# DrownFish19/PaddleXDE

Measured on AMD Instinct MI355X. Metric: integrated states/sec (batch*dim/step_time) dopri5, higher is better.
Workload: dtype f32

## Files before the change

paddlexde_amd/csrc/xde_seam.hip:

```cpp

#include "xde_common.hpp"
#include "xde_reduce.hpp"
#include "xde_errnorm_device.hpp"
#include "xde_control_device.hpp"
#include "xde_hip_seam.h"

using namespace xde;

namespace {

constexpr int kSeamCap = XDE_SEAM_CAP;
constexpr int kSeamBatch = 4;
constexpr int kSeamBlocksPerCU = 2;
static_assert(kSeamCap % kSeamBatch == 0, "whole batches");

struct alignas(128) SeamLine {
  unsigned long long gen;
  unsigned long long pad[15];
};
struct SeamState {
  SeamLine line[kTicketShards];
  SeamLine expired;
};

struct SeamCtrl {
  xde_ctrl_t* ctrl;
  xde_ctrl_params_t p;
  const double* t_span;
  const double* step_t;
  void* t_stage_out;
  xde_ctrl_t* mirror;
  int flags;
};

struct SeamArgs {
  ErrArgs e;
  const void* f0[2];
  void* out;
  double a21;
  SeamState* st;
  long long spin_limit;
};

template <typename T, int NORM, bool NT>
__global__ __launch_bounds__(kBlock, kSeamBlocksPerCU) void xde_seam_kernel(SeamArgs s, SeamCtrl tl) {
  __shared__ double seg_val[XDE_MAX_SEG];
  __shared__ double seg_nf[XDE_MAX_SEG];
  __shared__ xde_ctrl_t zs;
  __shared__ TimePrefetch pfs;
  __shared__ xde_ctrl_t sink;
  __shared__ double t_sink[XDE_MAX_STAGE];
  __shared__ int s_expired;
  using P = Pack<T, true>;
  constexpr int W = P::W;
  const ErrArgs& a = s.e;
  const bool pub = blockIdx.x == 0;
  control_prologue(tl.ctrl, tl.p, tl.t_span, tl.step_t, pub ? tl.mirror : nullptr, tl.flags, &zs, &pfs);

  const T* epre = static_cast<const T*>(a.e_pre);
  const T* __restrict__ kl = static_cast<const T*>(a.k[0]);
  const T* __restrict__ y1 = static_cast<const T*>(a.y1);
  const int64_t start = a.map.seg_start[0];
  const int64_t len = a.map.seg_len[0];
  const int64_t nvec = len / W;
  const int64_t vbase = start / W;
  const int64_t stride = int64_t(gridDim.x) * kBlock;
  const int64_t b0 = int64_t(blockIdx.x) * kBlock;
  const int64_t i0 = b0 + threadIdx.x;
  const double dtd = __builtin_nontemporal_load(&a.ctrl->dt);
  const int32_t accw = __builtin_nontemporal_load(&a.ctrl->accept);
  unsigned long long prior = 0;
  if (threadIdx.x == 0) prior = __hip_atomic_load(&s.st->expired.gen, __ATOMIC_RELAXED, __HIP_MEMORY_SCOPE_AGENT);
  const T rtol = T(a.rtol), atol = T(a.atol);
  const int sel = (a.use_sel && accw) ? 1 : 0;
  const T* __restrict__ y0 = static_cast<const T*>(a.y0[sel]);
  const T c = T(dtd) * T(a.coef[0]);
  T acc = T(0);
  int nfw = 0;
  P cy[kSeamCap], ck[kSeamCap];
  auto one = [&](bool on, T e, T y0e, T y1e) {
    T tol = atol + rtol * fmax_(abs_(y0e), abs_(y1e));
    T ar = abs_(e / tol);
    if (on) {
      if (NORM == XDE_NORM_RMS) {
        acc = acc + ar * ar;
      } else {
        acc = (ar != ar || acc != acc) ? (ar != ar ? ar : acc) : (ar > acc ? ar : acc);
      }
    }
    nfw += __popcll(__ballot(on && nonfinite_class(y0e)));
  };
#pragma unroll
  for (int jb = 0; jb < kSeamCap; jb += kSeamBatch) {
    if (b0 + int64_t(jb) * stride < nvec) {
      P ep[kSeamBatch], yv[kSeamBatch];
#pragma unroll
      for (int u = 0; u < kSeamBatch; ++u) {
        const int64_t i = i0 + int64_t(jb + u) * stride;
        const int64_t ic = vbase + (i < nvec ? i : nvec - 1);
        cy[jb + u] = P::load(y1, ic);
        ep[u] = NT ? P::load_nt(epre, ic) : P::load(epre, ic);
        ck[jb + u] = P::load(kl, ic);
        yv[u] = NT ? P::load_nt(y0, ic) : P::load(y0, ic);
      }
#pragma unroll
      for (int u = 0; u < kSeamBatch; ++u) {
        const bool on = i0 + int64_t(jb + u) * stride < nvec;
#pragma unroll
        for (int w = 0; w < W; ++w) one(on, ep[u].v[w] + ck[jb + u].v[w] * c, yv[u].v[w], cy[jb + u].v[w]);
      }
    }
  }
  const int64_t tj = start + nvec * W + threadIdx.x;
  const bool ton = blockIdx.x == 0 && tj < start + len;
  T ty1 = T(1), tk = T(0);
  if (blockIdx.x == 0) {
    T e = T(0), y0e = T(0);
    if (ton) {
      tk = kl[tj];
      e = epre[tj] + tk * c;
      y0e = y0[tj];
      ty1 = y1[tj];
    }
    if (ton) {
      T tol = atol + rtol * fmax_(abs_(y0e), abs_(ty1));
      T ar = abs_(e / tol);
      if (NORM == XDE_NORM_RMS) acc = acc + ar * ar;
      else acc = (ar != ar || acc != acc) ? (ar != ar ? ar : acc) : (ar > acc ? ar : acc);
    }
    nfw += __popcll(__ballot(ton && nonfinite_class(y0e)));
  }
  const double acc_d = NORM == XDE_NORM_RMS ? 0.0 + double(acc) : double(acc);
  const double nf_d = (threadIdx.x & 63) == 0 ? double(nfw) : 0.0;
  if (blockIdx.x == 0 && threadIdx.x == 0) {
    a.slot->nblocks = gridDim.x;
    a.slot->n_seg = 1;
    a.slot->norm_kind = NORM;
  }
  const bool last = block_reduce_store<NORM, true>(acc_d, nf_d, a.slot, 0);

  const unsigned long long tag = (unsigned long long)(zs.seq + 1);
  if (last) {
    if (threadIdx.x < kTicketShards)
      __hip_atomic_store(&a.slot->shard[threadIdx.x].count, 0u, __ATOMIC_RELAXED, __HIP_MEMORY_SCOPE_AGENT);
    if (threadIdx.x == 0) __hip_atomic_store(&a.slot->ticket, 0u, __ATOMIC_RELAXED, __HIP_MEMORY_SCOPE_AGENT);
    if (threadIdx.x < kTicketShards)
      __hip_atomic_store(&s.st->line[threadIdx.x].gen, tag, __ATOMIC_RELAXED, __HIP_MEMORY_SCOPE_AGENT);
  }
  if (threadIdx.x == 0) {
    int expired = prior != 0 ? 1 : 0;
    if (!last) {
      const unsigned nsh = gridDim.x < unsigned(kTicketShards) ? gridDim.x : unsigned(kTicketShards);
      const unsigned long long* word = &s.st->line[blockIdx.x % nsh].gen;
      long long spins = 0;
      while (__hip_atomic_load(word, __ATOMIC_RELAXED, __HIP_MEMORY_SCOPE_AGENT) != tag) {
        if (++spins > s.spin_limit) {
          expired = 1;
          unsigned long long none = 0;
          __hip_atomic_compare_exchange_strong(&s.st->expired.gen, &none, tag, __ATOMIC_RELAXED, __ATOMIC_RELAXED,
                                               __HIP_MEMORY_SCOPE_AGENT);
          break;
        }
        __builtin_amdgcn_s_sleep(8);
      }
    }
    s_expired = expired;
  }
  if (threadIdx.x < XDE_MAX_SEG) {
    seg_val[threadIdx.x] = 0.0;
    seg_nf[threadIdx.x] = 0.0;
  }
  __syncthreads();

  reduce_partials<true>(a.slot, seg_val, seg_nf, int(gridDim.x), 1, NORM);
  if (threadIdx.x == 0 && s_expired) seg_nf[0] += 1.0;
  __syncthreads();
  control_tail(pub ? tl.ctrl : &sink, tl.p, seg_val, seg_nf, tl.t_span, tl.step_t, pub ? tl.t_stage_out : static_cast<void*>(t_sink),
               pub ? tl.mirror : nullptr, tl.flags, &zs, &pfs);
  const int acc_new = zs.accept;
  const T c1 = T(s.a21) * T(zs.dt);
  T* out = static_cast<T*>(s.out);
  if (acc_new) {
#pragma unroll
    for (int j = 0; j < kSeamCap; ++j) {
      const int64_t i = i0 + int64_t(j) * stride;
      if (i < nvec) {
        P o;
#pragma unroll
        for (int w = 0; w < W; ++w) o.v[w] = cy[j].v[w] + ck[j].v[w] * c1;
        o.store(out, vbase + i);
      }
    }
    if (ton) out[tj] = ty1 + tk * c1;
  } else {
    const T* __restrict__ fb = static_cast<const T*>(s.f0[sel]);
    for (int64_t i = i0; i < nvec; i += stride) {
      P y = P::load(y0, vbase + i);
      P f = P::load(fb, vbase + i);
      P o;
#pragma unroll
      for (int w = 0; w < W; ++w) o.v[w] = y.v[w] + f.v[w] * c1;
      o.store(out, vbase + i);
    }
    if (ton) out[tj] = y0[tj] + fb[tj] * c1;
  }
}

template <typename T, int NORM, bool NT>
int seam_resident() {
  static int cache[64];
  static std::mutex mu;
  int dev = 0;
  if (hipGetDevice(&dev) != hipSuccess || dev < 0 || dev >= 64) {
    (void)hipGetLastError();
    return 0;
  }
  std::lock_guard<std::mutex> lk(mu);
  if (cache[dev] == 0) {
    int per_cu = 0, cus = 0;
    if (hipOccupancyMaxActiveBlocksPerMultiprocessor(&per_cu, xde_seam_kernel<T, NORM, NT>, kBlock, 0) != hipSuccess ||
        hipDeviceGetAttribute(&cus, hipDeviceAttributeMultiprocessorCount, dev) != hipSuccess) {
      (void)hipGetLastError();
      return 0;
    }
    if (per_cu > kSeamBlocksPerCU) per_cu = kSeamBlocksPerCU;
    cache[dev] = per_cu * cus > 0 ? per_cu * cus : -1;
  }
  return cache[dev] > 0 ? cache[dev] : 0;
}

int seam_resident_of(int dtype, int norm_kind, bool nt) {
#define SEAM_RES(T, NORM) (nt ? seam_resident<T, NORM, true>() : seam_resident<T, NORM, false>())
  if (dtype == XDE_F32) return norm_kind == XDE_NORM_RMS ? SEAM_RES(float, XDE_NORM_RMS) : SEAM_RES(float, XDE_NORM_LINF);
  return norm_kind == XDE_NORM_RMS ? SEAM_RES(double, XDE_NORM_RMS) : SEAM_RES(double, XDE_NORM_LINF);
#undef SEAM_RES
}

int seam_geometry(int64_t n, int dtype, int* blocks_out, int* per_lane_out) {
  xde_segments_t segs;
  memset(&segs, 0, sizeof(segs));
  segs.struct_size = sizeof(segs);
  segs.n_seg = 1;
  segs.seg_len[0] = n;
  const int width = dtype == XDE_F32 ? 4 : 2;
  SegMap m;
  int blocks = 0;
  if (int rc = build_segmap(&segs, width, true, &m, &blocks)) return rc;
  const int64_t nvec = n / width;
  const int64_t lanes = int64_t(blocks) * kBlock;
  *blocks_out = blocks;
  *per_lane_out = int((nvec + lanes - 1) / lanes);
  return XDE_OK;
}

}

extern "C" {

int64_t xde_seam_state_bytes(void) { return int64_t(sizeof(SeamState)); }

int xde_seam_plan(int64_t n, int dtype, xde_seam_plan_t* plan_out) {
  if (!plan_out) return fail(XDE_EBADARG, "xde_seam_plan: null pointer");
  if (dtype != XDE_F32 && dtype != XDE_F64) return fail(XDE_EBADARG, "xde_seam_plan: bad dtype");
  if (n < 1) return fail(XDE_EBADARG, "xde_seam_plan: n must be positive");
  memset(plan_out, 0, sizeof(*plan_out));
  int blocks = 0, per_lane = 0;
  if (int rc = seam_geometry(n, dtype, &blocks, &per_lane)) return rc;
  plan_out->blocks = blocks;
  plan_out->per_lane = per_lane;
  int resident = seam_resident_of(dtype, XDE_NORM_RMS, false);
  const int others[3] = {seam_resident_of(dtype, XDE_NORM_RMS, true), seam_resident_of(dtype, XDE_NORM_LINF, false),
                         seam_resident_of(dtype, XDE_NORM_LINF, true)};
  for (int r : others) resident = r < resident ? r : resident;
  plan_out->resident = resident;
  plan_out->fits = (blocks <= resident && per_lane <= kSeamCap) ? 1 : 0;
  return XDE_OK;
}

int xde_seam_attempt(const void* k_last, double c_last, const void* e_pre, const void* y0, const void* y0_alt, const void* f0,
                     const void* f0_alt, const void* y1, void* out, double a21, int64_t n, int dtype, void* ws, void* state,
                     xde_ctrl_t* ctrl, const xde_ctrl_params_t* params, const double* t_span_dev, const double* step_t_dev,
                     void* t_stage_out, xde_ctrl_t* host_mirror, int64_t spin_limit, void* stream) {
  if (!k_last || !e_pre || !y0 || !f0 || !y1 || !out || !ws || !state || !ctrl || !t_span_dev || !t_stage_out)
    return fail(XDE_EBADARG, "xde_seam_attempt: null pointer");
  int rc = check_params(params, "xde_seam_attempt");
  if (rc != XDE_OK) return rc;
  if (params->n_seg != 1) return fail(XDE_EBADARG, "xde_seam_attempt: one segment only");
  if (params->n_step_t > 0 && !step_t_dev) return fail(XDE_EBADARG, "xde_seam_attempt: n_step_t > 0 without step_t_dev");
  if (dtype != params->state_dtype) return fail(XDE_EBADARG, "xde_seam_attempt: dtype does not match params->state_dtype");
  if ((y0_alt == nullptr) != (f0_alt == nullptr)) return fail(XDE_EBADARG, "xde_seam_attempt: y0_alt/f0_alt must come together");
  if (n < 1) return fail(XDE_EBADARG, "xde_seam_attempt: n must be positive");
  if (spin_limit <= 0) return fail(XDE_EBADARG, "xde_seam_attempt: spin_limit must be positive (the wait is bounded)");
  xde_segments_t segs;
  memset(&segs, 0, sizeof(segs));
  segs.struct_size = sizeof(segs);
  segs.n_seg = 1;
  segs.seg_len[0] = n;
  SeamArgs s;
  memset(&s, 0, sizeof(s));
  bool vec = false;
  int nblocks = 0;
  double bytes = 0;
  const void* kk[1] = {k_last};
  rc = setup_err_args("xde_seam_attempt", kk, nullptr, &c_last, 1, y0, y0_alt, y1, params->rtol, params->atol, 0.0, ctrl, &segs,
                      params->norm_kind, dtype, ws, e_pre, &s.e, &vec, &nblocks, &bytes);
  if (rc != XDE_OK) return rc;
  vec = vec && aligned16(out) && aligned16(f0) && (!f0_alt || aligned16(f0_alt));
  if (!vec) return fail(XDE_EBADARG, "xde_seam_attempt: operands must be 16-byte aligned");
  const int width = dtype == XDE_F32 ? 4 : 2;
  const int64_t lanes = int64_t(nblocks) * kBlock;
  const int64_t per_lane = (n / width + lanes - 1) / lanes;
  const int resident = seam_resident_of(dtype, params->norm_kind, s.e.nt != 0);
  if (nblocks > resident || per_lane > kSeamCap)
    return fail(XDE_EBADARG, "xde_seam_attempt: the state does not fit the resident launch (" + std::to_string(nblocks) + " workgroups, " +
                                 std::to_string(resident) + " resident; " + std::to_string(per_lane) + " vectors per lane, " +
                                 std::to_string(kSeamCap) + " carried): take the separate launches");
  s.f0[0] = f0;
  s.f0[1] = f0_alt ? f0_alt : f0;
  s.out = out;
  s.a21 = a21;
  s.st = static_cast<SeamState*>(state);
  s.spin_limit = spin_limit;
  SeamCtrl tl;
  tl.ctrl = ctrl;
  tl.p = *params;
  tl.t_span = t_span_dev;
  tl.step_t = step_t_dev;
  tl.t_stage_out = t_stage_out;
  tl.mirror = host_mirror;
  tl.flags = ctrl_flags();
  hipStream_t st = static_cast<hipStream_t>(stream);
  ProfScope prof(XDE_KID_ERRNORM, 5.0 * double(n) * (dtype == XDE_F32 ? 4.0 : 8.0));
  dim3 g(nblocks), b(kBlock);
#define LAUNCH_SEAM(T, NORM)                                                   \
  do {                                                                         \
    if (s.e.nt)                                                                \
      XDE_LAUNCH((xde_seam_kernel<T, NORM, true>), g, b, st, prof, s, tl);     \
    else                                                                       \
      XDE_LAUNCH((xde_seam_kernel<T, NORM, false>), g, b, st, prof, s, tl);    \
  } while (0)
  if (dtype == XDE_F32) {
    if (params->norm_kind == XDE_NORM_RMS) LAUNCH_SEAM(float, XDE_NORM_RMS);
    else LAUNCH_SEAM(float, XDE_NORM_LINF);
  } else {
    if (params->norm_kind == XDE_NORM_RMS) LAUNCH_SEAM(double, XDE_NORM_RMS);
    else LAUNCH_SEAM(double, XDE_NORM_LINF);
  }
#undef LAUNCH_SEAM
  HIP_TRY(hipGetLastError());
  return XDE_OK;
}

int xde_seam_expired(const void* state, int64_t* tag_out, void* stream) {
  if (!state || !tag_out) return fail(XDE_EBADARG, "xde_seam_expired: null pointer");
  hipStream_t st = static_cast<hipStream_t>(stream);
  HIP_TRY(hipMemcpyAsync(tag_out, &static_cast<const SeamState*>(state)->expired.gen, sizeof(int64_t), hipMemcpyDeviceToHost, st));
  HIP_TRY(hipStreamSynchronize(st));
  return XDE_OK;
}

}
```

Before: 27.70 billion.

## Replace last-block ticket barrier with collector block publishing checksummed dt/accept

```diff
diff --git a/paddlexde_amd/csrc/xde_seam.hip b/paddlexde_amd/csrc/xde_seam.hip
--- a/paddlexde_amd/csrc/xde_seam.hip
+++ b/paddlexde_amd/csrc/xde_seam.hip
@@ -10,18 +10,38 @@
 namespace {
 
 constexpr int kSeamCap = XDE_SEAM_CAP;
-constexpr int kSeamBatch = 4;
+constexpr int kSeamPair = 1;
 constexpr int kSeamBlocksPerCU = 2;
-static_assert(kSeamCap % kSeamBatch == 0, "whole batches");
+constexpr int kSeamRecPer = 4;
+constexpr int kSeamCollectSleep = 1;
+static_assert(kSeamCap % kSeamPair == 0, "whole batches");
+static_assert(kSeamRecPer <= XDE_MAX_PARTIALS / kBlock, "the collector's records are reduce_records' first slots");
 
 struct alignas(128) SeamLine {
-  unsigned long long gen;
-  unsigned long long pad[15];
+  unsigned long long w[2];
+  unsigned long long pad[14];
 };
 struct SeamState {
   SeamLine line[kTicketShards];
   SeamLine expired;
 };
+
+__device__ __forceinline__ unsigned long long seam_chk(unsigned long long word, unsigned long long tag, int pos) {
+  return ctrl_mix64(word + 0x9E3779B97F4A7C15ull * (4ull * tag + (unsigned long long)pos));
+}
+
+__device__ __forceinline__ void seam_store_half(unsigned long long* at, unsigned long long word, unsigned long long tag, int pos) {
+  __hip_atomic_store(at + 0, word, __ATOMIC_RELAXED, __HIP_MEMORY_SCOPE_AGENT);
+  __hip_atomic_store(at + 1, seam_chk(word, tag, pos), __ATOMIC_RELAXED, __HIP_MEMORY_SCOPE_AGENT);
+}
+
+__device__ __forceinline__ void seam_load_half(const unsigned long long* at, unsigned long long& word, unsigned long long& check) {
+  typedef unsigned long long v2u64_t __attribute__((ext_vector_type(2)));
+  v2u64_t v;
+  asm volatile("global_load_dwordx4 %0, %1, off sc1\n\ts_waitcnt vmcnt(0)" : "=&v"(v) : "v"(at) : "memory");
+  word = v.x;
+  check = v.y;
+}
 
 struct SeamCtrl {
   xde_ctrl_t* ctrl;
@@ -48,14 +68,17 @@
   __shared__ double seg_nf[XDE_MAX_SEG];
   __shared__ xde_ctrl_t zs;
   __shared__ TimePrefetch pfs;
-  __shared__ xde_ctrl_t sink;
-  __shared__ double t_sink[XDE_MAX_STAGE];
-  __shared__ int s_expired;
+  __shared__ double s_val[kWaves];
+  __shared__ double s_nf[kWaves];
+  __shared__ int s_accept;
+  __shared__ int s_skip;
+  __shared__ unsigned long long s_dt;
+  __shared__ unsigned long long s_tag;
   using P = Pack<T, true>;
   constexpr int W = P::W;
   const ErrArgs& a = s.e;
   const bool pub = blockIdx.x == 0;
-  control_prologue(tl.ctrl, tl.p, tl.t_span, tl.step_t, pub ? tl.mirror : nullptr, tl.flags, &zs, &pfs);
+  if (pub) control_prologue(tl.ctrl, tl.p, tl.t_span, tl.step_t, tl.mirror, tl.flags, &zs, &pfs);
 
   const T* epre = static_cast<const T*>(a.e_pre);
   const T* __restrict__ kl = static_cast<const T*>(a.k[0]);
@@ -69,8 +92,11 @@
   const int64_t i0 = b0 + threadIdx.x;
   const double dtd = __builtin_nontemporal_load(&a.ctrl->dt);
   const int32_t accw = __builtin_nontemporal_load(&a.ctrl->accept);
-  unsigned long long prior = 0;
-  if (threadIdx.x == 0) prior = __hip_atomic_load(&s.st->expired.gen, __ATOMIC_RELAXED, __HIP_MEMORY_SCOPE_AGENT);
+  unsigned long long tag = 0, prior = 0;
+  if (threadIdx.x == 0) {
+    tag = (unsigned long long)(__builtin_nontemporal_load(&a.ctrl->seq) + 1);
+    prior = __hip_atomic_load(&s.st->expired.w[0], __ATOMIC_RELAXED, __HIP_MEMORY_SCOPE_AGENT);
+  }
   const T rtol = T(a.rtol), atol = T(a.atol);
   const int sel = (a.use_sel && accw) ? 1 : 0;
   const T* __restrict__ y0 = static_cast<const T*>(a.y0[sel]);
@@ -90,26 +116,45 @@
     }
     nfw += __popcll(__ballot(on && nonfinite_class(y0e)));
   };
-#pragma unroll
-  for (int jb = 0; jb < kSeamCap; jb += kSeamBatch) {
-    if (b0 + int64_t(jb) * stride < nvec) {
-      P ep[kSeamBatch], yv[kSeamBatch];
-#pragma unroll
-      for (int u = 0; u < kSeamBatch; ++u) {
-        const int64_t i = i0 + int64_t(jb + u) * stride;
-        const int64_t ic = vbase + (i < nvec ? i : nvec - 1);
-        cy[jb + u] = P::load(y1, ic);
-        ep[u] = NT ? P::load_nt(epre, ic) : P::load(epre, ic);
-        ck[jb + u] = P::load(kl, ic);
-        yv[u] = NT ? P::load_nt(y0, ic) : P::load(y0, ic);
-      }
-#pragma unroll
-      for (int u = 0; u < kSeamBatch; ++u) {
-        const bool on = i0 + int64_t(jb + u) * stride < nvec;
-#pragma unroll
-        for (int w = 0; w < W; ++w) one(on, ep[u].v[w] + ck[jb + u].v[w] * c, yv[u].v[w], cy[jb + u].v[w]);
-      }
-    }
+  P ep[2][kSeamPair], yv[2][kSeamPair];
+  auto live = [&](int jb) { return b0 + int64_t(jb) * stride < nvec; };
+  auto request = [&](int jb, int h) {
+#pragma unroll
+    for (int u = 0; u < kSeamPair; ++u) {
+      const int64_t i = i0 + int64_t(jb + u) * stride;
+      const int64_t ic = vbase + (i < nvec ? i : nvec - 1);
+      cy[jb + u] = P::load(y1, ic);
+      ep[h][u] = NT ? P::load_nt(epre, ic) : P::load(epre, ic);
+      ck[jb + u] = P::load(kl, ic);
+      yv[h][u] = NT ? P::load_nt(y0, ic) : P::load(y0, ic);
+    }
+  };
+  auto consume = [&](int jb, int h) {
+#pragma unroll
+    for (int u = 0; u < kSeamPair; ++u) {
+      const bool on = i0 + int64_t(jb + u) * stride < nvec;
+#pragma unroll
+      for (int w = 0; w < W; ++w) one(on, ep[h][u].v[w] + ck[jb + u].v[w] * c, yv[h][u].v[w], cy[jb + u].v[w]);
+    }
+  };
+  auto from = [&](auto self, auto jbc) {
+    constexpr int JB = decltype(jbc)::value;
+    constexpr int H = (JB / kSeamPair) & 1;
+    if constexpr (JB + kSeamPair < kSeamCap) {
+      if (live(JB + kSeamPair)) {
+        request(JB + kSeamPair, H ^ 1);
+        consume(JB, H);
+        self(self, std::integral_constant<int, JB + kSeamPair>{});
+      } else {
+        consume(JB, H);
+      }
+    } else {
+      consume(JB, H);
+    }
+  };
+  if (live(0)) {
+    request(0, 0);
+    from(from, std::integral_constant<int, 0>{});
   }
   const int64_t tj = start + nvec * W + threadIdx.x;
   const bool ton = blockIdx.x == 0 && tj < start + len;
@@ -130,55 +175,132 @@
     }
     nfw += __popcll(__ballot(ton && nonfinite_class(y0e)));
   }
-  const double acc_d = NORM == XDE_NORM_RMS ? 0.0 + double(acc) : double(acc);
-  const double nf_d = (threadIdx.x & 63) == 0 ? double(nfw) : 0.0;
+  double rec_v = NORM == XDE_NORM_RMS ? 0.0 + double(acc) : double(acc);
+  double rec_f = (threadIdx.x & 63) == 0 ? double(nfw) : 0.0;
   if (blockIdx.x == 0 && threadIdx.x == 0) {
     a.slot->nblocks = gridDim.x;
     a.slot->n_seg = 1;
     a.slot->norm_kind = NORM;
   }
-  const bool last = block_reduce_store<NORM, true>(acc_d, nf_d, a.slot, 0);
-
-  const unsigned long long tag = (unsigned long long)(zs.seq + 1);
-  if (last) {
-    if (threadIdx.x < kTicketShards)
-      __hip_atomic_store(&a.slot->shard[threadIdx.x].count, 0u, __ATOMIC_RELAXED, __HIP_MEMORY_SCOPE_AGENT);
-    if (threadIdx.x == 0) __hip_atomic_store(&a.slot->ticket, 0u, __ATOMIC_RELAXED, __HIP_MEMORY_SCOPE_AGENT);
-    if (threadIdx.x < kTicketShards)
-      __hip_atomic_store(&s.st->line[threadIdx.x].gen, tag, __ATOMIC_RELAXED, __HIP_MEMORY_SCOPE_AGENT);
-  }
+#pragma unroll
+  for (int off = 32; off > 0; off >>= 1) {
+    rec_v = merge_<NORM>(rec_v, __shfl_down(rec_v, off, 64));
+    rec_f += __shfl_down(rec_f, off, 64);
+  }
+  if ((threadIdx.x & 63) == 0) {
+    s_val[threadIdx.x >> 6] = rec_v;
+    s_nf[threadIdx.x >> 6] = rec_f;
+  }
+  if (threadIdx.x < XDE_MAX_SEG) {
+    seg_val[threadIdx.x] = 0.0;
+    seg_nf[threadIdx.x] = 0.0;
+  }
+  __syncthreads();
   if (threadIdx.x == 0) {
-    int expired = prior != 0 ? 1 : 0;
-    if (!last) {
+    double v = s_val[0], f = s_nf[0];
+#pragma unroll
+    for (int w = 1; w < kWaves; ++w) {
+      v = merge_<NORM>(v, s_val[w]);
+      f += s_nf[w];
+    }
+    unsigned long long* r = reinterpret_cast<unsigned long long*>(&a.slot->p[blockIdx.x]);
+    seam_store_half(r + 0, (unsigned long long)__double_as_longlong(v), tag, 0);
+    seam_store_half(r + 2, (unsigned long long)__double_as_longlong(f), tag, 1);
+    s_tag = tag;
+  }
+
+  int acc_new = 0;
+  double dt_new = 0.0;
+  if (pub) {
+    __syncthreads();
+    const unsigned long long tg = s_tag;
+    constexpr int kPer = XDE_MAX_PARTIALS / kBlock;
+    double rv[kPer], rf[kPer];
+    int rs[kPer];
+#pragma unroll
+    for (int i = 0; i < kPer; ++i) {
+      rv[i] = 0.0;
+      rf[i] = 0.0;
+      rs[i] = (i < kSeamRecPer && int(threadIdx.x) + i * kBlock < int(gridDim.x)) ? 0 : -1;
+    }
+    unsigned have = 0;
+    int expired = 0;
+    for (long long spins = 0;;) {
+      unsigned long long q[kSeamRecPer][4];
+#pragma unroll
+      for (int i = 0; i < kSeamRecPer; ++i) {
+        if (rs[i] == 0 && !(have >> i & 1u)) {
+          const unsigned long long* r = reinterpret_cast<const unsigned long long*>(&a.slot->p[threadIdx.x + i * kBlock]);
+#pragma unroll
+          for (int k = 0; k < 4; ++k) q[i][k] = __hip_atomic_load(r + k, __ATOMIC_RELAXED, __HIP_MEMORY_SCOPE_AGENT);
+        }
+      }
+      bool ok = true;
+#pragma unroll
+      for (int i = 0; i < kSeamRecPer; ++i) {
+        if (rs[i] == 0 && !(have >> i & 1u)) {
+          if (q[i][1] == seam_chk(q[i][0], tg, 0) && q[i][3] == seam_chk(q[i][2], tg, 1)) {
+            rv[i] = __longlong_as_double((long long)q[i][0]);
+            rf[i] = __longlong_as_double((long long)q[i][2]);
+            have |= 1u << i;
+          } else {
+            ok = false;
+          }
+        }
+      }
+      if (__syncthreads_and(ok ? 1 : 0)) break;
+      if (++spins > s.spin_limit) {
+        expired = 1;
+        break;
+      }
+      __builtin_amdgcn_s_sleep(kSeamCollectSleep);
+    }
+    reduce_records(rv, rf, rs, 1, NORM == XDE_NORM_RMS, seg_val, seg_nf);
+    if (threadIdx.x == 0) {
+      if (expired) {
+        unsigned long long none = 0;
+        __hip_atomic_compare_exchange_strong(&s.st->expired.w[0], &none, tg, __ATOMIC_RELAXED, __ATOMIC_RELAXED, __HIP_MEMORY_SCOPE_AGENT);
+      }
+      if (expired || prior != 0) seg_nf[0] += 1.0;
+    }
+    __syncthreads();
+    control_tail(tl.ctrl, tl.p, seg_val, seg_nf, tl.t_span, tl.step_t, tl.t_stage_out, tl.mirror, tl.flags, &zs, &pfs);
+    acc_new = zs.accept;
+    dt_new = zs.dt;
+    const int nsh = int(gridDim.x) < kTicketShards ? int(gridDim.x) : kTicketShards;
+    const int gl = int(threadIdx.x) - 64;
+    if (gl >= 0 && gl < nsh && gridDim.x > 1)
+      seam_store_half(s.st->line[gl].w, (unsigned long long)__double_as_longlong(dt_new), tg, acc_new ? 3 : 2);
+  } else {
+    if (threadIdx.x == 0) {
       const unsigned nsh = gridDim.x < unsigned(kTicketShards) ? gridDim.x : unsigned(kTicketShards);
-      const unsigned long long* word = &s.st->line[blockIdx.x % nsh].gen;
-      long long spins = 0;
-      while (__hip_atomic_load(word, __ATOMIC_RELAXED, __HIP_MEMORY_SCOPE_AGENT) != tag) {
-        if (++spins > s.spin_limit) {
-          expired = 1;
+      const unsigned long long* g = s.st->line[blockIdx.x % nsh].w;
+      int skip = 0, verdict = 0;
+      unsigned long long q[2];
+      for (long long spins = 0;;) {
+        seam_load_half(g, q[0], q[1]);
+        verdict = q[1] == seam_chk(q[0], tag, 3) ? 1 : 0;
+        if (verdict || q[1] == seam_chk(q[0], tag, 2)) break;
+        if (++spins > 2 * s.spin_limit) {
+          skip = 1;
           unsigned long long none = 0;
-          __hip_atomic_compare_exchange_strong(&s.st->expired.gen, &none, tag, __ATOMIC_RELAXED, __ATOMIC_RELAXED,
+          __hip_atomic_compare_exchange_strong(&s.st->expired.w[0], &none, tag, __ATOMIC_RELAXED, __ATOMIC_RELAXED,
                                                __HIP_MEMORY_SCOPE_AGENT);
           break;
         }
         __builtin_amdgcn_s_sleep(8);
       }
-    }
-    s_expired = expired;
-  }
-  if (threadIdx.x < XDE_MAX_SEG) {
-    seg_val[threadIdx.x] = 0.0;
-    seg_nf[threadIdx.x] = 0.0;
-  }
-  __syncthreads();
-
-  reduce_partials<true>(a.slot, seg_val, seg_nf, int(gridDim.x), 1, NORM);
-  if (threadIdx.x == 0 && s_expired) seg_nf[0] += 1.0;
-  __syncthreads();
-  control_tail(pub ? tl.ctrl : &sink, tl.p, seg_val, seg_nf, tl.t_span, tl.step_t, pub ? tl.t_stage_out : static_cast<void*>(t_sink),
-               pub ? tl.mirror : nullptr, tl.flags, &zs, &pfs);
-  const int acc_new = zs.accept;
-  const T c1 = T(s.a21) * T(zs.dt);
+      s_accept = verdict;
+      s_dt = q[0];
+      s_skip = skip;
+    }
+    __syncthreads();
+    if (s_skip) return;
+    acc_new = s_accept;
+    dt_new = __longlong_as_double((long long)s_dt);
+  }
+
+  const T c1 = T(s.a21) * T(dt_new);
   T* out = static_cast<T*>(s.out);
   if (acc_new) {
 #pragma unroll
@@ -224,7 +346,9 @@
       return 0;
     }
     if (per_cu > kSeamBlocksPerCU) per_cu = kSeamBlocksPerCU;
-    cache[dev] = per_cu * cus > 0 ? per_cu * cus : -1;
+    int res = per_cu * cus;
+    if (res > kSeamRecPer * kBlock) res = kSeamRecPer * kBlock;
+    cache[dev] = res > 0 ? res : -1;
   }
   return cache[dev] > 0 ? cache[dev] : 0;
 }
@@ -354,7 +478,7 @@
 int xde_seam_expired(const void* state, int64_t* tag_out, void* stream) {
   if (!state || !tag_out) return fail(XDE_EBADARG, "xde_seam_expired: null pointer");
   hipStream_t st = static_cast<hipStream_t>(stream);
-  HIP_TRY(hipMemcpyAsync(tag_out, &static_cast<const SeamState*>(state)->expired.gen, sizeof(int64_t), hipMemcpyDeviceToHost, st));
+  HIP_TRY(hipMemcpyAsync(tag_out, &static_cast<const SeamState*>(state)->expired.w[0], sizeof(int64_t), hipMemcpyDeviceToHost, st));
   HIP_TRY(hipStreamSynchronize(st));
   return XDE_OK;
 }
```

Result: no change. 27.59 billion (-0.4%).
